# ucla-mobility/QuantV2X

Measured on AMD Instinct MI355X. Metric: frames/sec/node (N-agent int8 BEV fusion), higher is better.
Workload: dtype i8

## Files before the change

quantv2x_amd/csrc/pfn_scatter.hip:

```cpp
#include "common.h"

namespace qv2x {

constexpr int PFN_PB = 4, PFN_PQ = 2;

__global__ __launch_bounds__(256, 6) void pfn_scatter_kernel(const float4* __restrict__ vf, const int4* __restrict__ coords,
                                                          const int* __restrict__ npts, int M, int P,
                                                          const qv2x_pfn_params prm, int8_t* __restrict__ canvas,
                                                          int N, int ny, int nx) {
    const int lane = threadIdx.x & 63;
    int m0 = (blockIdx.x * 4 + (threadIdx.x >> 6)) * PFN_PB;
    m0 = __builtin_amdgcn_readfirstlane(m0);
    if (m0 >= M) return;

    int4 c[PFN_PB];
    int np[PFN_PB];
    float4 q[PFN_PB][PFN_PQ];
#pragma unroll
    for (int j = 0; j < PFN_PB; ++j) {
        const int m = m0 + j < M ? m0 + j : M - 1;
        c[j] = coords[m];
        np[j] = npts[m];
    }
#pragma unroll
    for (int j = 0; j < PFN_PB; ++j) {
        const int m = m0 + j < M ? m0 + j : M - 1;
#pragma unroll
        for (int p = 0; p < PFN_PQ; ++p) q[j][p] = vf[(size_t)m * P + (p < P ? p : P - 1)];
    }
    float w[10];
#pragma unroll
    for (int k = 0; k < 10; ++k) w[k] = prm.w[lane * 10 + k];
    const float b = prm.b[lane];

#pragma unroll
    for (int j = 0; j < PFN_PB; ++j) {
        if (m0 + j >= M) break;
        const float4* pts = vf + (size_t)(m0 + j) * P;
        const int real = np[j] < P ? np[j] : P;
        float sx = 0.f, sy = 0.f, sz = 0.f;
#pragma unroll
        for (int p = 0; p < PFN_PQ; ++p)
            if (p < real) { sx += q[j][p].x; sy += q[j][p].y; sz += q[j][p].z; }
        for (int p = PFN_PQ; p < real; ++p) {
            const float4 t = pts[p];
            sx += t.x; sy += t.y; sz += t.z;
        }
        const float n = (float)np[j];
        const float mx = sx / n, my = sy / n, mz = sz / n;
        const float cx = (float)c[j].w * prm.vox[0] + prm.off[0];
        const float cy = (float)c[j].z * prm.vox[1] + prm.off[1];
        const float cz = (float)c[j].y * prm.vox[2] + prm.off[2];

        float ymax = -INFINITY;
        auto point = [&](const float4 t) __attribute__((always_inline)) {
            const float f[10] = {t.x, t.y, t.z, t.w, t.x - mx, t.y - my, t.z - mz, t.x - cx, t.y - cy, t.z - cz};
            float acc = 0.0f;
#pragma unroll
            for (int k = 0; k < 10; ++k) acc = fmaf(f[k], w[k], acc);
            ymax = fmaxf(ymax, acc + b);
        };
#pragma unroll
        for (int p = 0; p < PFN_PQ; ++p)
            if (p < real) point(q[j][p]);
        for (int p = PFN_PQ; p < real; ++p) point(pts[p]);
        if (real < P) ymax = fmaxf(ymax, b);

        const float q1 = q_code(ymax, prm.d1, prm.z1);
        float y1 = (q1 - prm.z1) * prm.d1;
        y1 = fmaxf(y1, 0.0f);
        const int code = (int)q_code(y1, prm.d2, prm.z2);

        if (c[j].x < 0 || c[j].x >= N || c[j].z < 0 || c[j].z >= ny || (c[j].y + c[j].w) < 0 || (c[j].y + c[j].w) >= nx) continue;
        const size_t cell = ((size_t)c[j].x * (ny + 2) + (c[j].z + 1)) * (nx + 2) + (size_t)(c[j].y + c[j].w + 1);
        canvas[cell * 64 + lane] = (int8_t)(code - 128);
    }
}

constexpr int PFN_R = 8;
#ifndef PFN_NQ
#define PFN_NQ 2
#endif

__global__ __launch_bounds__(256, 4) void pfn_scatter16_kernel(const float4* __restrict__ vf, const int4* __restrict__ coords,
                                                            const int* __restrict__ npts, int M, int P,
                                                            const qv2x_pfn_params prm, int8_t* __restrict__ canvas,
                                                            int N, int ny, int nx, int rounds) {
    __shared__ float wl[640 + 64];
    __shared__ uint8_t lut[256];
    for (int i = threadIdx.x; i < 640; i += 256) wl[i] = prm.w[i];
    if (threadIdx.x < 64) wl[640 + threadIdx.x] = prm.b[threadIdx.x];
    {
        const float q1 = (float)(threadIdx.x ^ 0x80);
        float y1 = (q1 - prm.z1) * prm.d1;
        y1 = fmaxf(y1, 0.0f);
        lut[threadIdx.x] = (uint8_t)((int)q_code(y1, prm.d2, prm.z2) - 128);
    }
    const float rd1 = 1.0f / prm.d1;
    __syncthreads();
    const int sub = threadIdx.x & 15, slot = threadIdx.x >> 4;
    float w[4][10], b[4];
#pragma unroll
    for (int c = 0; c < 4; ++c) {
#pragma unroll
        for (int k = 0; k < 10; ++k) w[c][k] = wl[(sub * 4 + c) * 10 + k];
        b[c] = wl[640 + sub * 4 + c];
    }
    const int mbase = blockIdx.x * (16 * rounds) + slot;

    auto header = [&](int m, int4& c, int& np, float4 (&q)[PFN_NQ]) __attribute__((always_inline)) {
        const int mm = m < M ? m : M - 1;
        c = coords[mm];
        np = npts[mm];
#pragma unroll
        for (int p = 0; p < PFN_NQ; ++p) q[p] = vf[(size_t)mm * P + (p < P ? p : P - 1)];
    };
    int4 c, cn;
    int np, npn;
    float4 q[PFN_NQ], qn[PFN_NQ];
    header(mbase, c, np, q);
#pragma unroll 1
    for (int r = 0; r < rounds; ++r) {
        const int m = mbase + r * 16;
        if (r + 1 < rounds) header(m + 16, cn, npn, qn);
        if (m < M) {
            const float4* pts = vf + (size_t)m * P;
            const int real = np < P ? np : P;
            float sx = 0.f, sy = 0.f, sz = 0.f;
#pragma unroll
            for (int p = 0; p < PFN_NQ; ++p)
                if (p < real) { sx += q[p].x; sy += q[p].y; sz += q[p].z; }
            for (int p = PFN_NQ; p < real; ++p) {
                const float4 t = pts[p];
                sx += t.x; sy += t.y; sz += t.z;
            }
            const float n = (float)np;
            const float mx = sx / n, my = sy / n, mz = sz / n;
            const float cx = (float)c.w * prm.vox[0] + prm.off[0];
            const float cy = (float)c.z * prm.vox[1] + prm.off[1];
            const float cz = (float)c.y * prm.vox[2] + prm.off[2];
            float ymax[4] = {-INFINITY, -INFINITY, -INFINITY, -INFINITY};
            auto point = [&](const float4 t) __attribute__((always_inline)) {
                const float f[10] = {t.x, t.y, t.z, t.w, t.x - mx, t.y - my, t.z - mz, t.x - cx, t.y - cy, t.z - cz};
#pragma unroll
                for (int ch = 0; ch < 4; ++ch) {
                    float acc = 0.0f;
#pragma unroll
                    for (int k = 0; k < 10; ++k) acc = fmaf(f[k], w[ch][k], acc);
                    ymax[ch] = fmaxf(ymax[ch], acc + b[ch]);
                }
            };
#pragma unroll
            for (int p = 0; p < PFN_NQ; ++p)
                if (p < real) point(q[p]);
            for (int p = PFN_NQ; p < real; ++p) point(pts[p]);
            if (real < P) {
#pragma unroll
                for (int ch = 0; ch < 4; ++ch) ymax[ch] = fmaxf(ymax[ch], b[ch]);
            }
            const unsigned c1 = (unsigned)q_pack4_div(ymax[0], ymax[1], ymax[2], ymax[3], prm.d1, rd1, prm.z1);
            const unsigned word = (unsigned)lut[c1 & 0xff] | ((unsigned)lut[(c1 >> 8) & 0xff] << 8) | ((unsigned)lut[(c1 >> 16) & 0xff] << 16) |
                                  ((unsigned)lut[c1 >> 24] << 24);
            if (!(c.x < 0 || c.x >= N || c.z < 0 || c.z >= ny || (c.y + c.w) < 0 || (c.y + c.w) >= nx)) {
                const size_t cell = ((size_t)c.x * (ny + 2) + (c.z + 1)) * (nx + 2) + (size_t)(c.y + c.w + 1);
                *(unsigned*)(canvas + cell * 64 + sub * 4) = word;
            }
        }
        c = cn; np = npn;
#pragma unroll
        for (int p = 0; p < PFN_NQ; ++p) q[p] = qn[p];
    }
}

__global__ __launch_bounds__(256) void pfn_unscatter_kernel(const int4* __restrict__ coords, int M, int value4, int8_t* __restrict__ canvas,
                                                            int N, int ny, int nx) {
    const long long id = (long long)blockIdx.x * 256 + threadIdx.x;
    const int m = (int)(id >> 2), piece = (int)(id & 3);
    if (m >= M) return;
    const int4 c = coords[m];
    if (c.x < 0 || c.x >= N || c.z < 0 || c.z >= ny || (c.y + c.w) < 0 || (c.y + c.w) >= nx) return;
    const size_t cell = ((size_t)c.x * (ny + 2) + (c.z + 1)) * (nx + 2) + (size_t)(c.y + c.w + 1);
    v4i v; v[0] = v[1] = v[2] = v[3] = value4;
    *(v4i*)(canvas + cell * 64 + piece * 16) = v;
}

}

extern "C" int qv2x_pfn_unscatter_i8(const int32_t* voxel_coords, int M, int value, int8_t* canvas, int N, int ny, int nx, void* stream) {
    using namespace qv2x;
    if (M == 0) return QV2X_OK;
    if (!voxel_coords || !canvas) return fail(QV2X_EINVAL, "qv2x_pfn_unscatter_i8: null pointer");
    if (M < 0 || N <= 0 || ny <= 0 || nx <= 0 || value < -128 || value > 127) return fail(QV2X_EINVAL, "qv2x_pfn_unscatter_i8: bad sizes / value");
    if (((uintptr_t)voxel_coords & 15) || ((uintptr_t)canvas & 15)) return fail(QV2X_EALIGN, "qv2x_pfn_unscatter_i8: coords / canvas must be 16-byte aligned");
    const int b = value & 0xff, v4 = b | (b << 8) | (b << 16) | (b << 24);
    const long long threads = (long long)M * 4;
    pfn_unscatter_kernel<<<(unsigned)((threads + 255) / 256), 256, 0, (hipStream_t)stream>>>((const int4*)voxel_coords, M, v4, canvas, N, ny, nx);
    return hip_check(hipGetLastError(), "qv2x_pfn_unscatter_i8 launch");
}

extern "C" int qv2x_pfn_scatter_i8(const float* voxel_features, const int32_t* voxel_coords, const int32_t* voxel_num_points,
                                   int M, int max_points, const qv2x_pfn_params* params, int8_t* canvas, int N, int ny, int nx,
                                   void* stream) {
    using namespace qv2x;
    if (M == 0) return QV2X_OK;
    if (!voxel_features || !voxel_coords || !voxel_num_points || !params || !canvas)
        return fail(QV2X_EINVAL, "qv2x_pfn_scatter_i8: null pointer");
    if (M < 0 || max_points <= 0 || N <= 0 || ny <= 0 || nx <= 0) return fail(QV2X_EINVAL, "qv2x_pfn_scatter_i8: bad sizes");
    if (((uintptr_t)voxel_features & 15) || ((uintptr_t)voxel_coords & 15)) return fail(QV2X_EALIGN, "qv2x_pfn_scatter_i8: inputs must be 16-byte aligned");
    int form = 16;
#ifdef QV2X_DEV_KNOBS
    static const int form_env = getenv("QV2X_PFN_FORM") ? atoi(getenv("QV2X_PFN_FORM")) : 16;
    form = form_env;
#endif
    if (form == 64)
        pfn_scatter_kernel<<<(M + 4 * PFN_PB - 1) / (4 * PFN_PB), 256, 0, (hipStream_t)stream>>>((const float4*)voxel_features, (const int4*)voxel_coords,
                                                                         voxel_num_points, M, max_points, *params, canvas, N, ny, nx);
    else {
        static const int cus = [] {
            int dev = 0, v = 0;
            return hipGetDevice(&dev) == hipSuccess && hipDeviceGetAttribute(&v, hipDeviceAttributeMultiprocessorCount, dev) == hipSuccess && v > 0 ? v : 256;
        }();
        int rounds = M / (16 * 8 * cus);
        rounds = rounds < 1 ? 1 : (rounds > PFN_R ? PFN_R : rounds);
        pfn_scatter16_kernel<<<(M + 16 * rounds - 1) / (16 * rounds), 256, 0, (hipStream_t)stream>>>((const float4*)voxel_features, (const int4*)voxel_coords,
                                                                          voxel_num_points, M, max_points, *params, canvas, N, ny, nx, rounds);
    }
    return hip_check(hipGetLastError(), "qv2x_pfn_scatter_i8 launch");
}
```

Measured before the change: 6675.

## Add MFMA-based PFN scatter kernel for large pillar counts

```diff
diff --git a/quantv2x_amd/csrc/pfn_scatter.hip b/quantv2x_amd/csrc/pfn_scatter.hip
--- a/quantv2x_amd/csrc/pfn_scatter.hip
+++ b/quantv2x_amd/csrc/pfn_scatter.hip
@@ -172,6 +172,127 @@
     }
 }
 
+constexpr int PFN_MR = 8, PFN_MFMA_MIN_PILLARS = 80000;
+
+__device__ __forceinline__ float pfn_max(float a, float b, float inf) { return __builtin_amdgcn_fmed3f(a, b, inf); }
+__device__ __forceinline__ float pfn_pair(float v) {
+    return __builtin_bit_cast(float, __builtin_amdgcn_update_dpp(0, __builtin_bit_cast(int, v), 0xB1, 0xf, 0xf, false));
+}
+
+__global__ __launch_bounds__(256, 4) void pfn_scatter_mfma_kernel(const float4* __restrict__ vf, const int4* __restrict__ coords,
+                                                               const int* __restrict__ npts, int M, int P,
+                                                               const qv2x_pfn_params prm, int8_t* __restrict__ canvas,
+                                                               int N, int ny, int nx, int rounds) {
+    __shared__ uint8_t lut[256];
+    __shared__ float bl[64];
+    if (threadIdx.x < 64) bl[threadIdx.x] = prm.b[threadIdx.x];
+    {
+        const float q1 = (float)(threadIdx.x ^ 0x80);
+        float y1 = (q1 - prm.z1) * prm.d1;
+        y1 = fmaxf(y1, 0.0f);
+        lut[threadIdx.x] = (uint8_t)((int)q_code(y1, prm.d2, prm.z2) - 128);
+    }
+    const float rd1 = 1.0f / prm.d1;
+    __syncthreads();
+    const int lane = threadIdx.x & 63, wave = threadIdx.x >> 6;
+    const int h = lane >> 5, s = lane & 1, ch0 = 32 * s + 4 * h;
+    float wa[2][5];
+#pragma unroll
+    for (int tile = 0; tile < 2; ++tile)
+#pragma unroll
+        for (int t = 0; t < 5; ++t) wa[tile][t] = prm.w[((lane & 31) + 32 * tile) * 10 + 2 * t + h];
+    const int mbase = blockIdx.x * (64 * rounds) + wave * 16 + ((lane & 31) >> 1);
+    float inf = INFINITY;
+    asm volatile("" : "+v"(inf));
+
+    auto header = [&](int m, int4& c, int& np, float4& q0, float4& q1) __attribute__((always_inline)) {
+        const int mm = m < M ? m : M - 1;
+        c = coords[mm];
+        np = npts[mm];
+        q0 = vf[(size_t)mm * P];
+        q1 = vf[(size_t)mm * P + 1];
+    };
+    int4 c, cn;
+    int np, npn;
+    float4 q0, q1, q0n, q1n;
+    header(mbase, c, np, q0, q1);
+    cn = c; npn = np; q0n = q0; q1n = q1;
+#pragma unroll 1
+    for (int r = 0; r < rounds; ++r) {
+        const int m = mbase + r * 64;
+        if (__builtin_amdgcn_readfirstlane(m - ((lane & 31) >> 1)) >= M) break;
+        if (r + 1 < rounds) header(m + 64, cn, npn, q0n, q1n);
+        const float4* pts = vf + (size_t)(m < M ? m : M - 1) * P;
+        const int real = np < P ? np : P;
+        float sx = 0.f, sy = 0.f, sz = 0.f;
+        if (0 < real) { sx += q0.x; sy += q0.y; sz += q0.z; }
+        if (1 < real) { sx += q1.x; sy += q1.y; sz += q1.z; }
+        constexpr int PFN_MS = 4;
+        for (int p = 2; __builtin_amdgcn_ballot_w64(p < real) != 0; p += PFN_MS) {
+            float tx[PFN_MS], ty[PFN_MS], tz[PFN_MS];
+#pragma unroll
+            for (int i = 0; i < PFN_MS; ++i) {
+                const float* t = (const float*)(pts + (p + i < real ? p + i : 0));
+                tx[i] = t[0]; ty[i] = t[1]; tz[i] = t[2];
+            }
+#pragma unroll
+            for (int i = 0; i < PFN_MS; ++i)
+                if (p + i < real) { sx += tx[i]; sy += ty[i]; sz += tz[i]; }
+        }
+        const float n = (float)np;
+        const float s2 = (h ? sy : sx) / n, mz = sz / n;
+        const float cx = (float)c.w * prm.vox[0] + prm.off[0];
+        const float cy = (float)c.z * prm.vox[1] + prm.off[1];
+        const float cz = (float)c.y * prm.vox[2] + prm.off[2];
+        const float s3 = h ? cx : mz, s4 = h ? cz : cy;
+        v16f ymax0, ymax1;
+#pragma unroll
+        for (int i = 0; i < 16; ++i) { ymax0[i] = -INFINITY; ymax1[i] = -INFINITY; }
+        float4 t = s ? q1 : q0;
+        bool live = s < real;
+        for (int p = 0;;) {
+            const bool more = __builtin_amdgcn_ballot_w64(p + 2 < real) != 0;
+            const bool liven = p + 2 + s < real || real == P;
+            float4 tn = t;
+            if (more) tn = pts[p + 2 + s < real ? p + 2 + s : (real == P ? P - 1 : 0)];
+            const float a = h ? t.y : t.x;
+            const float f[5] = {live ? a : 0.0f, live ? (h ? t.w : t.z) : 0.0f, live ? a - s2 : 0.0f,
+                                live ? (h ? t.x : t.z) - s3 : 0.0f, live ? (h ? t.z : t.y) - s4 : 0.0f};
+            v16f a0, a1;
+#pragma unroll
+            for (int i = 0; i < 16; ++i) { a0[i] = 0.0f; a1[i] = 0.0f; }
+#pragma unroll
+            for (int t5 = 0; t5 < 5; ++t5) {
+                a0 = __builtin_amdgcn_mfma_f32_32x32x2f32(wa[0][t5], f[t5], a0, 0, 0, 0);
+                a1 = __builtin_amdgcn_mfma_f32_32x32x2f32(wa[1][t5], f[t5], a1, 0, 0, 0);
+            }
+#pragma unroll
+            for (int i = 0; i < 16; ++i) { ymax0[i] = pfn_max(ymax0[i], a0[i], inf); ymax1[i] = pfn_max(ymax1[i], a1[i], inf); }
+            if (!more) break;
+            t = tn; live = liven; p += 2;
+        }
+        float y[16];
+#pragma unroll
+        for (int i = 0; i < 16; ++i) y[i] = pfn_max(s ? ymax1[i] : ymax0[i], pfn_pair(s ? ymax0[i] : ymax1[i]), inf);
+        const bool inside = m < M && !(c.x < 0 || c.x >= N || c.z < 0 || c.z >= ny || (c.y + c.w) < 0 || (c.y + c.w) >= nx);
+        const size_t cell = ((size_t)c.x * (ny + 2) + (c.z + 1)) * (nx + 2) + (size_t)(c.y + c.w + 1);
+#pragma unroll
+        for (int j = 0; j < 4; ++j) {
+            float yj[4];
+#pragma unroll
+            for (int i = 0; i < 4; ++i) {
+                const float b = bl[ch0 + 8 * j + i];
+                yj[i] = pfn_max(y[4 * j + i] + b, real < P ? b : -INFINITY, inf);
+            }
+            const unsigned c1 = (unsigned)q_pack4_div(yj[0], yj[1], yj[2], yj[3], prm.d1, rd1, prm.z1);
+            const unsigned word = (unsigned)lut[c1 & 0xff] | ((unsigned)lut[(c1 >> 8) & 0xff] << 8) | ((unsigned)lut[(c1 >> 16) & 0xff] << 16) |
+                                  ((unsigned)lut[c1 >> 24] << 24);
+            if (inside) *(unsigned*)(canvas + cell * 64 + ch0 + 8 * j) = word;
+        }
+        c = cn; np = npn; q0 = q0n; q1 = q1n;
+    }
+}
+
 __global__ __launch_bounds__(256) void pfn_unscatter_kernel(const int4* __restrict__ coords, int M, int value4, int8_t* __restrict__ canvas,
                                                             int N, int ny, int nx) {
     const long long id = (long long)blockIdx.x * 256 + threadIdx.x;
@@ -207,19 +328,27 @@
         return fail(QV2X_EINVAL, "qv2x_pfn_scatter_i8: null pointer");
     if (M < 0 || max_points <= 0 || N <= 0 || ny <= 0 || nx <= 0) return fail(QV2X_EINVAL, "qv2x_pfn_scatter_i8: bad sizes");
     if (((uintptr_t)voxel_features & 15) || ((uintptr_t)voxel_coords & 15)) return fail(QV2X_EALIGN, "qv2x_pfn_scatter_i8: inputs must be 16-byte aligned");
-    int form = 16;
+    int form = max_points >= 2 && M >= PFN_MFMA_MIN_PILLARS ? 32 : 16;
+    int mfma_div = 16;
 #ifdef QV2X_DEV_KNOBS
-    static const int form_env = getenv("QV2X_PFN_FORM") ? atoi(getenv("QV2X_PFN_FORM")) : 16;
-    form = form_env;
+    static const int form_env = getenv("QV2X_PFN_FORM") ? atoi(getenv("QV2X_PFN_FORM")) : 0;
+    static const int div_env = getenv("QV2X_PFN_MFMA_DIV") ? atoi(getenv("QV2X_PFN_MFMA_DIV")) : 0;
+    if (form_env == 64 || form_env == 16 || (form_env == 32 && max_points >= 2)) form = form_env;
+    if (div_env > 0) mfma_div = div_env;
 #endif
+    static const int cus = [] {
+        int dev = 0, v = 0;
+        return hipGetDevice(&dev) == hipSuccess && hipDeviceGetAttribute(&v, hipDeviceAttributeMultiprocessorCount, dev) == hipSuccess && v > 0 ? v : 256;
+    }();
     if (form == 64)
         pfn_scatter_kernel<<<(M + 4 * PFN_PB - 1) / (4 * PFN_PB), 256, 0, (hipStream_t)stream>>>((const float4*)voxel_features, (const int4*)voxel_coords,
                                                                          voxel_num_points, M, max_points, *params, canvas, N, ny, nx);
-    else {
-        static const int cus = [] {
-            int dev = 0, v = 0;
-            return hipGetDevice(&dev) == hipSuccess && hipDeviceGetAttribute(&v, hipDeviceAttributeMultiprocessorCount, dev) == hipSuccess && v > 0 ? v : 256;
-        }();
+    else if (form == 32) {
+        int rounds = M / (64 * mfma_div * cus);
+        rounds = rounds < 1 ? 1 : (rounds > PFN_MR ? PFN_MR : rounds);
+        pfn_scatter_mfma_kernel<<<(M + 64 * rounds - 1) / (64 * rounds), 256, 0, (hipStream_t)stream>>>((const float4*)voxel_features, (const int4*)voxel_coords,
+                                                                             voxel_num_points, M, max_points, *params, canvas, N, ny, nx, rounds);
+    } else {
         int rounds = M / (16 * 8 * cus);
         rounds = rounds < 1 ? 1 : (rounds > PFN_R ? PFN_R : rounds);
         pfn_scatter16_kernel<<<(M + 16 * rounds - 1) / (16 * rounds), 256, 0, (hipStream_t)stream>>>((const float4*)voxel_features, (const int4*)voxel_coords,
```

Result: slower. 6510 (-2.5%).
